# ohseokkwon/Foveated-Rendering-using-Ray-Tracing

Measured on AMD Instinct MI355X. Metric: Mrays/s + reconstructed fps @4K, 10% foveal density, 1/2/4/8 GPU, higher is better.
Workload: dtype f32

## Files before the change

### foveated-rendering-using-ray-tracing_amd/csrc/ctx_create.cpp

```cpp
#include <cmath>
#include <cstdlib>

#include "ctx_internal.h"

using namespace fr;
using fri::fail;

static thread_local std::string g_create_error;

int fri::fail(fr_ctx* c, int code, const std::string& msg) {
  if (c) c->err = msg; else g_create_error = msg;
  return code;
}

extern "C" {

const char* fr_version(void) { return "fovrt 0.2 (gfx950)"; }
int fr_abi_version(void) { return FOVRT_ABI_VERSION; }

int fr_config_default(fr_config* c) {
  if (!c) return FR_E_INVALID;
  memset(c, 0, sizeof(*c));
  c->abi_version = FOVRT_ABI_VERSION;
  c->width = 1024; c->height = 1024;
// ... 33 lines not shown
    const float M = std::max(v[0], std::max(v[1], v[2]));
    uint32_t word = 0;
    if (M > 0.0f) {
      int ex = 0;
      std::frexp(M, &ex);
      const int k = ex - 8, e = k + 136;
      if (e < 1 || e > 255) return FR_TEX_F32;
      const float f = std::ldexp(1.0f, e - 136);
      for (int c = 0; c < 3; c++) {
        const float m = std::ldexp(v[c], -k);
        if (!(m >= 0.0f && m <= 255.0f) || m != std::floor(m) || !same((float)(int)m * f, v[c])) return FR_TEX_F32;
        word |= (uint32_t)m << (8 * c);
      }
      word |= (uint32_t)e << 24;
    } else if (!(same(v[0], 0.0f) && same(v[1], 0.0f) && same(v[2], 0.0f))) {
      return FR_TEX_F32;
    }
    out[i] = word;
  }
  return FR_TEX_RGBE;
}

static void read_env_knobs(fr_ctx* c) {
  if (const char* v = getenv("FOVRT_SHADE_CHUNK_REFR")) c->chunk_refr = (uint32_t)std::max(0, atoi(v));
  if (const char* v = getenv("FOVRT_SHADE_XCD_BANDS")) c->xcd_bands = atoi(v) != 0;
  if (const char* v = getenv("FOVRT_SHADE_HANDOFF")) c->handoff = (uint32_t)std::min(std::max(atoi(v), 0), 2);
  if (const char* v = getenv("FOVRT_TEX_PACKING")) c->tex_packing = atoi(v) != 0;
  if (const char* v = getenv("FOVRT_JFA_LAZY_OUTPUTS")) c->lazy_jfa_outputs = atoi(v) != 0;
  if (const char* v = getenv("FOVRT_EARLY_SETUP")) c->early_setup = atoi(v) != 0;
  if (const char* v = getenv("FOVRT_EXTRA_LAZY")) c->extra_lazy = atoi(v) != 0;
  if (const char* v = getenv("FOVRT_SIB_STRIP")) c->sib_strip = atoi(v) != 0;
  if (const char* v = getenv("FOVRT_SLOTS")) c->nslots = std::max(2, std::min(fr_ctx::MAX_SLOTS, atoi(v)));
  {
    const char* v = getenv("FOVRT_SHADE_BLOCKS_PER_CU");
    const int full = fr::shade_max_blocks_per_cu();
    c->shade_blocks_per_cu = v ? std::max(1, std::min(full, atoi(v))) : full;
  }
  if (const char* v = getenv("FOVRT_JFA_XCD")) c->jfa_xcd = atoi(v);
  if (const char* v = getenv("FOVRT_JFA_REUSE")) c->jfa_reuse = atoi(v) != 0;
  if (const char* v = getenv("FOVRT_SIB_STRIP_MID")) c->sib_strip_mid = atoi(v);
  if (const char* v = getenv("FOVRT_ATROUS_ROWS2")) c->atrous_rows2 = atoi(v) != 0;
  if (const char* v = getenv("FOVRT_ATROUS_XCD")) c->atrous_xcd = atoi(v) != 0;
  if (const char* v = getenv("FOVRT_RAYQ_BLOCKS")) c->rayq_blocks = (uint32_t)std::max(0, atoi(v));
}

static std::vector<hipEvent_t*> timed_events(fr_ctx* c) {
  fr_ctx::StageEvents& t = c->tev;
  std::vector<hipEvent_t*> v = {&t.begin, &t.geometry, &t.sampling, &t.optimize, &t.shading, &t.end, &t.paths_begin,
                                &t.paths_end, &t.chain2_begin, &t.pullpush, &t.atrous, &t.chain1_begin, &t.jfa,
                                &t.sibson, &t.stage_begin, &t.stage_end, &c->ev_carry_fork, &c->ev_carry_done,
                                &c->ev_recon_fork, &c->ev_chain2_done, &c->ev_stream_join};
  for (auto& s : c->lat.ev)
    for (hipEvent_t* e : {&s.front_begin, &s.front_end, &s.jfa_end, &s.recon_end}) v.push_back(e);
  return v;
}

int fr_create(const fr_config* cfg_in, fr_ctx** out) {
  if (!out) return fail(nullptr, FR_E_INVALID, "out is NULL");
  *out = nullptr;
  fr_config cfg;
  if (cfg_in) cfg = *cfg_in; else fr_config_default(&cfg);
  if (cfg.abi_version != FOVRT_ABI_VERSION)
    return fail(nullptr, FR_E_INVALID, "fr_config.abi_version != FOVRT_ABI_VERSION (initialise it with fr_config_default)");
  if (cfg.width <= 0 || cfg.height <= 0 || cfg.width > 32767 || cfg.height > 32767)
    return fail(nullptr, FR_E_INVALID, "width/height out of range (1..32767)");
  if (!(cfg.spp == 1 || cfg.spp == 2 || cfg.spp == 4 || cfg.spp == 8))
    return fail(nullptr, FR_E_UNSUPPORTED, "spp must be 1, 2, 4 or 8");
  if (cfg.mask_mode < 0 || cfg.mask_mode > 4) return fail(nullptr, FR_E_INVALID, "bad mask_mode");
// ... 348 lines not shown
```

### foveated-rendering-using-ray-tracing_amd/csrc/ctx_frame.cpp

```cpp
#include <immintrin.h>
#include <sched.h>

#include <chrono>
#include <cmath>
#include <functional>

#include "ctx_internal.h"

using namespace fr;
using namespace fri;

namespace {
constexpr float kPollDeadlineMs = 10000.0f;
inline void cpu_relax() { _mm_pause(); }
hipError_t poll_event(hipEvent_t ev, float deadline_ms) {
  const auto t0 = std::chrono::steady_clock::now();
  for (uint32_t n = 1;; n++) {
    const hipError_t e = hipEventQuery(ev);
    if (e != hipErrorNotReady) return e;
    if ((n & 63u) == 0) {
      if (std::chrono::duration<float, std::milli>(std::chrono::steady_clock::now() - t0).count() > deadline_ms)
        return hipErrorNotReady;
      sched_yield();
    } else {
// ... 161 lines not shown
    if (int rc = enqueue_optimize(c, c->stream)) return rc;
  }
  c->front_done.consume(c->stream);
  hipEvent_t* kt = nullptr;
  if (c->kt_on) {
    const int i = c->kt_next;
    if (c->kt_pending == fr_ctx::KT_RING) { kt_harvest(c, i); c->kt_pending--; }
    kt = c->kt_ev[i];
    c->kt_next = (i + 1) % fr_ctx::KT_RING;
    c->kt_pending++;
    hipEventRecord(kt[0], c->stream);
  }
  if (c->setup_early) {
    c->aux_i ^= 1;
    c->aux = c->aux_p[c->aux_i];
    c->aux_seed = c->aux_seed_p[c->aux_i];
  }
  const bool early = c->setup_early;
  c->setup_early = false;
  const bool hv = c->pipeline_mode == FR_PIPELINE_LATENCY && c->early_setup && c->U.shard_count <= 1 && !c->U.front_need;
  hipEventRecord(c->ev_carry_fork, c->stream);
  hipStreamWaitEvent(c->carry_stream, c->ev_carry_fork, 0);
  launch_carry_history(c->U, c->mask, c->img[P_wgt(c)], c->img[c->hist_cache], c->img[c->hist_cur],
                       c->img[P_shd(c)], hv ? c->hvalid : nullptr, c->carry_stream);
  hipEventRecord(c->ev_carry_done, c->carry_stream);
  const uint32_t N = (uint32_t)((size_t)c->W * c->H);
  if (!early)
    launch_sample_setup(c->U, c->active, c->ray_count, N, c->img[P_wgt(c)], c->img[c->hist_cache], nullptr, c->aux,
                        c->aux_seed, c->stream);
  if (c->time_kernels) hipEventRecord(c->tev.paths_begin, c->stream);
  if (kt) hipEventRecord(kt[1], c->stream);
  launch_shade_paths(c->dsc, c->U, c->active, c->ray_count, N, c->img[P_wgt(c)], c->img[c->hist_cache],
                     c->shade_ctr, c->samples, c->sample_help, c->stats, c->aux, c->aux_seed, c->chunk_refr,
                     c->xcd_bands, c->handoff, c->shade_blocks_per_cu, c->item_store, c->stream);
  if (c->time_kernels) hipEventRecord(c->tev.paths_end, c->stream);
  if (kt) hipEventRecord(kt[2], c->stream);
  hipStreamWaitEvent(c->stream, c->ev_carry_done, 0);
  launch_shade_resolve(c->U, c->active, c->ray_count, N, c->img[P_wgt(c)], c->img[c->hist_cache], c->samples,
                       c->sample_help, c->img[c->hist_cur], c->img[P_shd(c)], c->shade_ctr, c->handoff,
                       c->shade_blocks_per_cu, c->U.shard_count > 1 ? c->shade_radiance : nullptr, c->stream);
  if (kt) hipEventRecord(kt[3], c->stream);
  c->trace_done[c->slot].record(c->stream);
  mark_set_read(c);
  int rc = check_launch(c);
  std::swap(c->hist_cur, c->hist_cache);
  c->hvalid_fresh = hv;
  std::swap(c->depth_cur, c->depth_cache);
  return rc;
}

static void materialize_jfa(fr_ctx* c, hipStream_t s) {
  if (!c->jfa_coord_owed) return;
  launch_jfa_coord(c->jfa_final, c->img[P_JFA_COLOR], c->img[P_JFA_COORD], c->W, c->H, s);
  c->jfa_coord_owed = false;
}

void fr_ctx::ExtraDebt::record(const fr_ctx* c) {
  U = c->U;
  sc = c->dsc;
  box = c->dev_box;
  depth = c->depth_cur;
  nrm = P_nrm(c);
  wgt = P_wgt(c);
}
void fr_ctx::ExtraDebt::settle(fr_ctx* c) {
  if (!owed) return;
  join_recon(c);
// ... 356 lines not shown
```

### foveated-rendering-using-ray-tracing_amd/csrc/ctx_internal.h

```cpp
#pragma once
#include <hip/hip_runtime.h>

#include <cstring>
#include <string>
#include <vector>

#include "../../include/fovrt.h"
#include "fr_device.h"
#include "k_launch.h"
#include "scene.h"

#define FR_MAX_SHARD_RANKS 64

using fr::f2;
using fr::f3;
using fr::u2;
using fr::f4;
using fr::BvhNode;
using fr::TriGeo;
using fr::TriShade;
using fr::DevMaterial;
using fr::DevTexture;
using fr::DevScene;
using fr::DevStats;
// ... 146 lines not shown
  bool fov_dirty = true, fov_reset = true, fov_on_device = false;
  fr::FovState* fov_st = nullptr;
  fr::FovState* h_fov = nullptr;
  const uint32_t* fov_count = nullptr;
  uint8_t* cmask = nullptr;
  bool cmask_on = false, cmask_set = false;
  Fence mask_taken, mask_read;
  unsigned long long* words = nullptr;
  uint32_t* counts = nullptr;
  uint32_t* offsets = nullptr;
  uint32_t* tiles = nullptr;
  uint32_t* ray_count = nullptr;
  uint32_t* active = nullptr;
  uint32_t* shade_ctr = nullptr;
  f4* samples = nullptr;
  unsigned long long* sample_help = nullptr;
  f4* item_store = nullptr;
  f4* aux = nullptr;
  uint32_t* aux_seed = nullptr;
  f4* aux_p[2] = {};
  uint32_t* aux_seed_p[2] = {};
  int aux_i = 0;
  unsigned long long* hvalid = nullptr;
  bool hvalid_fresh = false;
  bool setup_early = false;
  bool early_setup = true;
  fr::JfaState jfa = {};
  uint32_t jfa_gen = 0;
  bool jfa_force = true;
  bool jfa_reuse = true;
  uint32_t chunk_refr = 0;
  uint32_t xcd_bands = 1;
  uint32_t handoff = 1;
  int shade_blocks_per_cu = 0;
  int jfa_xcd = 1;
  int sib_strip_mid = 0;
  bool atrous_rows2 = true;
  int atrous_xcd = 1;
  float* ftab = nullptr;
  f4 *pull = nullptr, *push = nullptr, *snap = nullptr;
  f4 *sib_prefix = nullptr, *sib_blocks = nullptr;
  uint32_t* sib_wide = nullptr;
  uint32_t* sib_strips = nullptr;
  f4* sib_rowp = nullptr;
  bool sib_prefix_fresh = false;
  const u2* jfa_final = nullptr;
  bool jfa_coord_owed = false;
  bool lazy_jfa_outputs = true;
  struct ExtraDebt {
    bool owed = false;
    FrameUniforms U;
    DevScene sc;
    const float* box = nullptr;
    int depth = P_DEPTH_A, nrm = P_NORMAL, wgt = P_WEIGHT;
    void record(const fr_ctx* c);
    bool reads(int phys) const;
    void settle(fr_ctx* c);
  } extra;
  bool extra_lazy = true;
  int pp_S = 0;
  DevStats* stats = nullptr;
  FrameUniforms U;
  uint32_t accum = 0;
  bool light_pending = false;
  bool compacted = false;
  bool mask_dirty = false;
// ... 66 lines not shown
```

### foveated-rendering-using-ray-tracing_amd/csrc/k_launch.h

```cpp
#pragma once
#include <hip/hip_runtime.h>

#include <cstddef>
#include <cstdint>
#include <string>

#include "fr_device.h"

namespace fr {
void launch_gbuffer(const DevScene& sc, const FrameUniforms& U, f4* position, f4* normal, f4* depth, f4* diffuse,
                    f4* weight, uint8_t* gclass, DevStats* stats, const f3* cur_pos, const f3* prev_pos,
                    hipStream_t stream);
void launch_shade_paths(const DevScene& sc, const FrameUniforms& U, const uint32_t* active, const uint32_t* ray_count,
                        uint32_t max_active, const f4* weight, const f4* history_cache, uint32_t* chunk_ctr,
                        f4* samples, unsigned long long* help, DevStats* stats, f4* aux, uint32_t* aux_seed,
                        uint32_t chunk_refr, uint32_t xcd_bands, uint32_t handoff, int per_cu, f4* item_store,
                        hipStream_t stream);
int shade_max_blocks_per_cu();
size_t shade_item_store_f4(int per_cu);
void launch_sample_setup(const FrameUniforms& U, const uint32_t* active, const uint32_t* ray_count, uint32_t max_active,
                         const f4* weight, const f4* history_cache, const unsigned long long* hvalid, f4* aux,
                         uint32_t* aux_seed, hipStream_t stream);
void launch_shade_resolve(const FrameUniforms& U, const uint32_t* active, const uint32_t* ray_count,
                          uint32_t max_active, const f4* weight, const f4* history_cache, const f4* samples,
                          unsigned long long* help, f4* history_buffer, f4* shading, uint32_t* chunk_ctr,
                          uint32_t handoff, int per_cu, f4* radiance, hipStream_t stream);
size_t shade_counter_words();
size_t shade_fx_slots(uint32_t max_active, int spp, uint32_t handoff, int per_cu);
void launch_carry_history(const FrameUniforms& U, const uint8_t* mask, const f4* weight, const f4* history_cache,
                          f4* history_buffer, f4* shading, unsigned long long* hvalid, hipStream_t stream);
void launch_shard_pack_active(const uint32_t* active, const uint32_t* ray_count, uint32_t capacity, const f4* radiance,
                              f4* vals, uint32_t* idx, hipStream_t stream);
void launch_shard_unpack_active(const FrameUniforms& U, const f4* vals, const uint32_t* idx, uint32_t n, uint32_t npix,
                                const f4* weight, const f4* history_cache, f4* history_buffer, f4* shading,
                                hipStream_t stream);
void launch_vring_pack(const f4* hist, int W, int H, int T, const int32_t* tiles, int ntiles, uint32_t* out,
                       hipStream_t stream);
void launch_vring_unpack(const uint32_t* in, int W, int H, int T, const int32_t* tiles, int ntiles, f4* hist,
                         hipStream_t stream);
void launch_ray_queries(const DevScene& sc, const void* rays, const uint32_t* masks, uint32_t n, int kind, void* out,
                        RayQueryState* rq, const RayModels& rm, uint32_t max_blocks, hipStream_t stream);
#ifdef FR_STAMPS
void launch_trace_queries(const DevScene& sc, const f4* queries, uint32_t n, f4* hits, uint32_t* ctr,
                          hipStream_t stream, int kind);
void diag_record_queries(f4* buf, uint32_t cap, hipStream_t stream);
uint32_t diag_recorded_queries(hipStream_t stream);
void diag_sample_trace(uint32_t* srec, uint32_t scap, uint32_t* wrec, uint32_t wcap, hipStream_t stream);
#endif

void launch_sampling(const FrameUniforms& U, const DevScene& sc, const f4* position, const f4* depth,
                     const f4* depth_cache, f4* weight, const f4* normal, const f4* diffuse, f4* extra, uint8_t* mask,
// ... 139 lines not shown
```

### foveated-rendering-using-ray-tracing_amd/csrc/k_trace.hip

```cpp
#include <hip/hip_runtime.h>
#include <cstdlib>
#include "fr_device.h"
#include "k_launch.h"

namespace fr {

#ifndef TRACE_BLOCK
#define TRACE_BLOCK 128
#endif
#define BVH_STACK FR_BVH_STACK
#define ITEM_STACK 24

#ifdef FR_STAMPS
FR_DEV uint64_t stamp() {
  uint64_t t;
  __builtin_amdgcn_sched_barrier(0);
  asm volatile("s_memtime %0\n\ts_waitcnt lgkmcnt(0)" : "=s"(t)::"memory");
  __builtin_amdgcn_sched_barrier(0);
  return t;
}
#define STAMP(v) const uint64_t v = stamp()
#define STAMP_ADD(acc, v) acc += stamp() - v
#else
#define STAMP(v)
// ... 424 lines not shown
        long long sum;
        if (__builtin_add_overflow(old, v[k], &sum)) ovf |= v[k] > 0 ? 16u << k : 256u << k;
      }
    if ((flags & FX_NONFINITE) | ovf) atomicOr(rec + 3, (unsigned long long)((flags & FX_NONFINITE) | ovf));
  }
};
FR_DEV float fx_comp(long long v, unsigned long long fl, int k) {
  const bool nan = (fl >> k) & 1, pinf = (fl >> (4 + k)) & 1, ninf = (fl >> (8 + k)) & 1;
  if (nan || (pinf && ninf)) return __builtin_nanf("");
  if (pinf) return INFINITY;
  if (ninf) return -INFINITY;
  return (float)((double)v * (1.0 / FX_ONE));
}
FR_DEV f3 sample_value(const f4* samples, unsigned long long* help, uint32_t slot, bool fx) {
  if (!fx) return xyz(samples[slot]);
  const ulonglong2* r = reinterpret_cast<const ulonglong2*>(samples) + (size_t)slot * 2;
  const ulonglong2 r0 = r[0], r1 = r[1];
  long long v0 = (long long)r0.x, v1 = (long long)r0.y, v2 = (long long)r1.x;
  unsigned long long fl = r1.y;
  if (fl & FX_HELPED) {
    ulonglong2* h = reinterpret_cast<ulonglong2*>(help + (size_t)slot * 4);
    const ulonglong2 h0 = h[0], h1 = h[1];
    const long long hv[3] = {(long long)h0.x, (long long)h0.y, (long long)h1.x};
    if (__builtin_add_overflow(v0, hv[0], &v0)) fl |= hv[0] > 0 ? 16u : 256u;
    if (__builtin_add_overflow(v1, hv[1], &v1)) fl |= hv[1] > 0 ? 32u : 512u;
    if (__builtin_add_overflow(v2, hv[2], &v2)) fl |= hv[2] > 0 ? 64u : 1024u;
    fl |= h1.y;
    h[0] = make_ulonglong2(0ull, 0ull);
    h[1] = make_ulonglong2(0ull, 0ull);
  }
  return mk3(fx_comp(v0, fl, 0), fx_comp(v1, fl, 1), fx_comp(v2, fl, 2));
}

struct PathState {
  int n;
  ItemState it;
  SampleSum total;
  f3 qo, qd;
  float qtmax;
  bool qany;
  int phase;
  bool diffuse_kind, want_child;
  f3 Kd, pres, cdir, front;
  float pm, nDl, LnDl, Ldist, phong;
  uint32_t cseed, seed;
};

FR_DEV void path_begin(PathState& ps, f3 o, f3 d, uint32_t seed, Counters cnt) {
  ps.n = 0;
  ps.it = ItemState{mk3(1.0f), 0, 1.0f};
  ps.total.clear();
  ps.qo = o; ps.qd = d; ps.qtmax = INFINITY; ps.qany = false;
  ps.phase = PH_ITEM;
  ps.diffuse_kind = true; ps.want_child = false;
  ps.Kd = ps.pres = ps.cdir = ps.front = mk3(0.0f);
  ps.pm = 1.0f; ps.nDl = ps.LnDl = ps.Ldist = 0.0f; ps.phong = -1.0f;
  ps.cseed = 0; ps.seed = seed;
  cnt.inc(C_PRIMARY);
}

FR_DEV bool path_shade_step(const DevScene& sc, const FrameUniforms& U, PathState& ps, const ItemStack& items, Counters cnt,
                            const Hit& h, float atten, f3& total) {
  int& n = ps.n;
  ItemState& it = ps.it;
  f3& qo = ps.qo;
  f3& qd = ps.qd;
  float& qtmax = ps.qtmax;
  bool& qany = ps.qany;
  int& phase = ps.phase;
  bool& diffuse_kind = ps.diffuse_kind;
  bool& want_child = ps.want_child;
  f3& Kd = ps.Kd;
  f3& pres = ps.pres;
  f3& cdir = ps.cdir;
  f3& front = ps.front;
  float& pm = ps.pm;
  float& nDl = ps.nDl;
  float& LnDl = ps.LnDl;
  float& Ldist = ps.Ldist;
  float& phong = ps.phong;
  uint32_t& cseed = ps.cseed;
  const uint32_t seed = ps.seed;
  const f3 cutoff = mk3(0.34f, 0.55f, 0.85f);
  {
    bool pop = false;
    if (phase == PH_ITEM) {
      if (h.leaf < 0) {
        total += it.w * envmap_miss(sc, qd);
        pop = true;
      } else {
        SurfaceHit s = surface(sc, h, qo, qd);
        const int type = sc.mats[s.mat].type;
        Kd = kd_of(sc, s.mat, s.uv);
        if (type == MATL_REFRACTION) {
          const f3 hp = fma3(h.t, qd, qo);
          const f3 nrm = s.ns;
          const f3 i = qd;
          const f3 wk = it.w * Kd;
          float reflection = 1.0f;
          if (it.depth < U.refraction_max_depth) {
            int pushed = 0;
            Item child;
            f3 tdir;
            if (refract(tdir, i, nrm, 1.4f)) {
              float cos_theta = dotc(i, nrm);
              if (cos_theta < 0.0f) cos_theta = -cos_theta;
              else cos_theta = dotc(tdir, nrm);
              reflection = fresnel_schlick(cos_theta, 3.0f, 0.1f, 1.0f);
              float importance = it.importance * (1.0f - reflection) * luminance(mk3(1.0f));
              if (importance > 0.01f) {
                if (n < ITEM_STACK) { child = Item{hp, tdir, wk * ((1.0f - reflection) * mk3(1.0f)), it.depth + 1, importance}; pushed = 1; cnt.inc(C_REFR); }
                else cnt.inc(C_OVERFLOW);
              } else {
                total += wk * ((1.0f - reflection) * mk3(1.0f) * cutoff);
              }
            }
            f3 r = reflect(i, nrm);
            float importance = it.importance * reflection * luminance(mk3(1.0f));
            if (importance > 0.01f) {
              if (n + pushed < ITEM_STACK) {
                if (pushed) items.put(n++, child);
                child = Item{hp, r, wk * (reflection * mk3(1.0f)), it.depth + 1, importance};
                pushed = 1;
                cnt.inc(C_REFL);
              } else {
                cnt.inc(C_OVERFLOW);
              }
            } else {
              total += wk * (reflection * mk3(1.0f) * cutoff);
            }
            if (pushed) {
              it = ItemState{child.w, child.depth, child.importance};
              qo = child.o; qd = child.d; qtmax = INFINITY; qany = false;
              phase = PH_ITEM;
              return false;
            }
          } else {
            cnt.inc(C_TRUNC);
          }
          pop = true;
        } else {
          const f3 ff = faceforward_neg(s.ns, qd, s.ng);
          uint32_t sd = seed;
          const float z1 = rnd(sd);
          const float z2 = rnd(sd);
          front = s.front;
          LightSample ls = light_sample(sc, ff, front, z1, z2);
          nDl = ls.nDl; LnDl = ls.LnDl; Ldist = ls.Ldist;
          cseed = sd;
          diffuse_kind = type == MATL_DIFFUSE;
          if (diffuse_kind) {
            pm = 1.0f;
            want_child = it.depth < U.diffuse_max_depth - 1;
            if (want_child) cdir = onb_inverse_transform(ff, cosine_sample_hemisphere(z1, z2));
          } else {
            f3 H = normalizec(ls.L - qd);
            float nDh = dotc(ff, H);
            phong = nDh > 0.0f ? fx_pow(nDh, 88.0f) : -1.0f;
            const float rn = 0.05f;
            pm = fresnel_schlick(-dotc(ff, qd), 5.0f, rn, 1.0f);
            float importance = it.importance * luminance(mk3(pm));
            want_child = importance > 0.01f && it.depth < U.reflection_max_depth;
            if (want_child) cdir = reflect(qd, ff);
          }
          phase = PH_PARENT_SHADOW;
          if (nDl > 0.0f && LnDl > 0.0f) {
            cnt.inc(C_SHADOW);
            qo = front; qd = ls.L; qtmax = Ldist; qany = true;
            return false;
          }
          atten = 0.0f;
        }
      }
    }
    if (!pop && phase == PH_PARENT_SHADOW) {
      f3 S = mk3(0.0f);
      if (nDl > 0.0f && LnDl > 0.0f && atten > 0.0f) {
        const float weight = light_weight(sc, nDl, LnDl, Ldist);
        if (diffuse_kind) {
          S += sc.light_emission * weight * mk3(atten);
        } else {
          f3 Lc = sc.light_emission * weight * mk3(atten);
          S += Kd * nDl * Lc;
          if (phong >= 0.0f) S = fma3(Lc * mk3(1.0f), mk3(phong), S);
        }
      }
      pres = Kd * S;
      if (want_child) {
        cnt.inc(diffuse_kind ? C_BOUNCE : C_MIRROR);
        qo = front; qd = cdir; qtmax = INFINITY; qany = false;
        phase = PH_CHILD;
        return false;
      }
      total += it.w * pres;
      pop = true;
    } else if (!pop && phase == PH_CHILD) {
      bool lit = false;
      if (h.leaf >= 0) {
        SurfaceHit s = surface(sc, h, qo, qd);
        if (sc.mats[s.mat].type == MATL_DIFFUSE) {
          const f3 ff = faceforward_neg(s.ns, qd, s.ng);
          uint32_t sd = cseed;
          const float z1 = rnd(sd);
          const float z2 = rnd(sd);
          Kd = kd_of(sc, s.mat, s.uv);
          LightSample ls = light_sample(sc, ff, s.front, z1, z2);
          nDl = ls.nDl; LnDl = ls.LnDl; Ldist = ls.Ldist;
          if (nDl > 0.0f && LnDl > 0.0f) {
            cnt.inc(C_SHADOW);
            qo = s.front; qd = ls.L; qtmax = Ldist; qany = true;
            phase = PH_CHILD_SHADOW;
            lit = true;
          }
        }
      }
      if (lit) return false;
      total += it.w * (pres + mk3(pm) * mk3(0.0f));
      pop = true;
    } else if (!pop && phase == PH_CHILD_SHADOW) {
      f3 S = mk3(0.0f);
      if (atten > 0.0f) S += sc.light_emission * light_weight(sc, nDl, LnDl, Ldist) * mk3(atten);
      total += it.w * fma3(mk3(pm), Kd * S, pres);
      pop = true;
    }
    if (n == 0) return true;
    const Item nx = items.get(--n);
    it = ItemState{nx.w, nx.depth, nx.importance};
    qo = nx.o; qd = nx.d; qtmax = INFINITY; qany = false;
    phase = PH_ITEM;
    return false;
  }
}

FR_DEV bool path_shade(const DevScene& sc, const FrameUniforms& U, PathState& ps, const ItemStack& items, Counters cnt,
                       const Hit& h, float atten, bool fx) {
  f3 c = fx ? mk3(0.0f) : ps.total.as_float();
  const bool done = path_shade_step(sc, U, ps, items, cnt, h, atten, c);
  if (fx) ps.total.add(c);
  else ps.total.set_float(c);
  return done;
}

FR_DEV Hit trace_closest(const DevScene& sc, Stack st, f3 o, f3 d, float tmin, float tmax) {
  Hit h;
  float a;
  traverse(sc, st, o, d, tmin, tmax, false, h, a);
  return h;
}

FR_DEV void counters_begin(uint32_t* lds) {
  if (threadIdx.x < C_COUNT) lds[threadIdx.x] = 0;
  __syncthreads();
}
FR_DEV void counters_end(DevStats* stats, uint32_t* lds, bool gbuf) {
  __syncthreads();
  if (threadIdx.x < C_COUNT) {
    unsigned long long v = lds[threadIdx.x];
    if (v) {
      unsigned long long* dst;
      switch (threadIdx.x) {
        case C_PRIMARY: dst = gbuf ? &stats->gbuffer_primary : &stats->primary; break;
        case C_SHADOW: dst = &stats->shadow; break;
        case C_BOUNCE: dst = &stats->diffuse_bounce; break;
        case C_MIRROR: dst = &stats->mirror; break;
        case C_REFR: dst = &stats->refraction; break;
        case C_REFL: dst = &stats->reflection; break;
        case C_TRUNC: dst = &stats->truncated; break;
        default: dst = &stats->bvh_overflow; break;
      }
      atomicAdd(dst, v);
// ... 185 lines not shown
__device__ f4* g_rec = nullptr;
__device__ uint32_t g_rec_n = 0;
__device__ uint32_t g_rec_cap = 0;
FR_DEV void record_query(f3 o, f3 d, float tmax, bool any) {
  if (!g_rec) return;
  const uint32_t i = atomicAdd(&g_rec_n, 1u);
  if (i < g_rec_cap) {
    g_rec[2 * (size_t)i] = mk4(o, tmax);
    g_rec[2 * (size_t)i + 1] = mk4(d, any ? 1.0f : 0.0f);
  }
}
#define RECORD_QUERY(ps) record_query(ps.qo, ps.qd, ps.qtmax, ps.qany)
#else
#define RECORD_QUERY(ps)
#endif

#ifdef FR_STAMPS
__device__ uint32_t* g_srec = nullptr;
__device__ uint32_t g_srec_cap = 0;
__device__ uint32_t* g_wrec = nullptr;
__device__ uint32_t g_wrec_cap = 0;
FR_DEV uint32_t rtime() { return (uint32_t)__builtin_amdgcn_s_memrealtime(); }
#define DIAG(x) x
#else
#define DIAG(x)
#endif

#ifndef TRAV_UNROLL
#define TRAV_UNROLL 2
#endif
#ifndef SHADE_FIRST_STEP
#define SHADE_FIRST_STEP 1
#endif
#ifndef SHADE_WAVES
#define SHADE_WAVES 3
#endif
#ifndef SHADE_EXIT_T
#define SHADE_EXIT_T 8
#endif
#ifndef SHADE_EXIT_S
#define SHADE_EXIT_S 0
#endif
#ifndef SHADE_EXIT_REFR
#define SHADE_EXIT_REFR 20
#endif
__global__ __launch_bounds__(TRACE_BLOCK) __attribute__((amdgpu_waves_per_eu(SHADE_WAVES, SHADE_WAVES))) void k_shade_paths(DevScene sc, FrameUniforms U,
                                                             const uint32_t* __restrict__ active,
                                                             const uint32_t* __restrict__ ray_count,
                                                             const f4* __restrict__ weight,
                                                             const f4* __restrict__ history_cache,
                                                             uint32_t* __restrict__ chunk_ctr,
                                                             f4* __restrict__ samples, DevStats* stats,
                                                             const f4* __restrict__ aux,
                                                             const uint32_t* __restrict__ aux_seed,
                                                             uint32_t chunk_refr_fixed, uint32_t xcd_bands,
                                                             unsigned long long* __restrict__ help, uint32_t fx_below,
                                                             f4* __restrict__ item_store) {
  __shared__ int32_t lds_stack[BVH_STACK * TRACE_BLOCK];
  __shared__ uint32_t lds_cnt[C_COUNT];
  __shared__ BvhNode lds_root;
  Stack st{&lds_stack[threadIdx.x]};
  if (threadIdx.x < 32) reinterpret_cast<float*>(&lds_root)[threadIdx.x] = reinterpret_cast<const float*>(sc.nodes)[threadIdx.x];
  counters_begin(lds_cnt);
  Counters cnt{lds_cnt};
  const ItemStack items{item_store + (size_t)(blockIdx.x * TRACE_BLOCK + threadIdx.x) * 4, gridDim.x * TRACE_BLOCK * 4u};
  const uint32_t spp_shift = __builtin_ctz((uint32_t)U.spp);
  const uint32_t total = ray_count[0] * (uint32_t)U.spp;
  const uint32_t nrefr = min(ray_count[1] * (uint32_t)U.spp, total);
  const bool fx = total < fx_below;
  const uint32_t lanes = gridDim.x * TRACE_BLOCK;
  const uint32_t chunk_refr = chunk_refr_fixed ? chunk_refr_fixed
                              : total < 8 * lanes
                                  ? min(max(nrefr / (lanes / 64), 8u), (uint32_t)SHADE_CHUNK) & ~((uint32_t)U.spp - 1u)
                                  : SHADE_CHUNK;
  const uint32_t nsmall = (nrefr + chunk_refr - 1) / chunk_refr;
  const uint32_t nchunks = nsmall + (total - nrefr + SHADE_CHUNK - 1) / SHADE_CHUNK;
  uint32_t cb[5];
  cb[0] = 0; cb[4] = total;
#pragma unroll
  for (int c = 1; c < 4; c++) cb[c] = min(ray_count[c] * (uint32_t)U.spp, total);
  cb[1] = nrefr;
  auto part = [&](int c, uint32_t s) {
    const uint32_t len = (cb[c + 1] - cb[c]) >> spp_shift;
    return cb[c] + (uint32_t)(((uint64_t)len * s / SHADE_SHARDS) << spp_shift);
  };
  const uint32_t lane = threadIdx.x & 63;
  const float tmin = sc.scene_epsilon;
  const bool exit_early = SHADE_EXIT_T > 0 && (SHADE_EXIT_REFR == 0 || (!fx && (uint64_t)nrefr * SHADE_EXIT_REFR >= total));
  uint32_t shard = blockIdx.x & (SHADE_SHARDS - 1);
  uint32_t shards_left = SHADE_SHARDS;
  uint32_t q_next = 0, q_end = 0;
  int ls = L_IDLE;
  uint32_t slot = 0;
  PathState ps;
  TravState ts;
  uint64_t trav_cycles = 0, step_cycles = 0, refill_cycles = 0, total_cycles = 0;
#ifdef FR_STAMPS
  uint32_t n_visits = 0, n_wave_steps = 0;
  uint32_t d_q = 0, d_steps = 0, d_t0 = 0, w_done = 0;
  const uint32_t w_begin = rtime();
  uint32_t w_dry = 0;
#endif
  STAMP(t_begin);
  while (true) {
    STAMP(t_refill);
    unsigned long long idle = __ballot(ls == L_IDLE);
    while (idle && (q_next < q_end || shards_left)) {
      if (q_next >= q_end) {
        if (xcd_bands) {
        bool found = false;
        uint32_t j = 0;
        if (lane == 0) j = atomicAdd(&chunk_ctr[shard * SHADE_SHARD_STRIDE], 1u);
        j = __builtin_amdgcn_readfirstlane(j);
#pragma unroll
        for (int c = 0; c < 4; c++) {
          const uint32_t b = part(c, shard), e = part(c, shard + 1);
          const uint32_t ch = c == 0 ? chunk_refr : SHADE_CHUNK;
          const uint32_t n = (e - b + ch - 1) / ch;
          if (!found && j < n) {
            q_next = b + j * ch;
// ... 71 lines not shown
          ps.seed = xseed;
          trav_begin(ts, ps.qd, ps.qtmax);
          RECORD_QUERY(ps);
          DIAG(d_q = 1; d_steps = 0; d_t0 = rtime());
          ls = L_TRAV;
        }
      }
    }
    STAMP_ADD(refill_cycles, t_refill);
    if (!__ballot(ls != L_IDLE)) {
      if (!more) break;
      continue;
    }
    STAMP(t_tr);
    const bool traverse = !SHADE_FIRST_STEP || !__ballot(ls == L_READY);
    for (uint32_t pass = 0; traverse && __ballot(ls == L_TRAV) &&
                            (!exit_early || pass < SHADE_EXIT_S || __popcll(__ballot(ls == L_TRAV)) > SHADE_EXIT_T ||
                             !__ballot(ls == L_READY));
         pass++) {
#ifdef FR_STAMPS
      n_wave_steps++;
      if (ls == L_TRAV) n_visits++;
#endif
#pragma unroll
      for (int u = 0; u < TRAV_UNROLL; u++)
        if (ls == L_TRAV) {
          DIAG(d_steps++);
          if (trav_step(sc, st, ts, ps.qo, ps.qd, tmin, ps.qtmax, ps.qany)) ls = L_READY;
        }
    }
    STAMP_ADD(trav_cycles, t_tr);
    STAMP(t_step);
    if (ls == L_READY) {
      const bool fin = path_shade(sc, U, ps, items, cnt, ts.best, (float)ts.atten, fx);
      if (fin) {
        ps.total.flush(samples, help, slot, fx);
        ls = L_IDLE;
#ifdef FR_STAMPS
        if (g_srec && slot < g_srec_cap) {
          g_srec[4 * (size_t)slot] = d_q; g_srec[4 * (size_t)slot + 1] = d_steps;
          g_srec[4 * (size_t)slot + 2] = d_t0; g_srec[4 * (size_t)slot + 3] = rtime();
        }
        w_done++;
#endif
      } else {
        trav_begin(ts, ps.qd, ps.qtmax);
        RECORD_QUERY(ps);
        DIAG(d_q++);
        ls = L_TRAV;
        if (SHADE_FIRST_STEP && !root_hit(lds_root, ps.qo, ts.inv, tmin, ps.qtmax)) ls = L_READY;
      }
    }
    STAMP_ADD(step_cycles, t_step);
  }
  STAMP_ADD(total_cycles, t_begin);
#ifdef FR_STAMPS
  if (lane == 0) {
    atomicAdd(&stats->pad[0], (unsigned long long)total_cycles);
    atomicAdd(&stats->pad[1], (unsigned long long)refill_cycles);
    atomicAdd(&stats->pad[2], (unsigned long long)step_cycles);
    atomicAdd(&stats->pad[3], (unsigned long long)trav_cycles);
    atomicAdd(&stats->pad[5], (unsigned long long)n_wave_steps);
  }
  atomicAdd(&stats->pad[4], (unsigned long long)n_visits);
  {
    const uint32_t wid = (blockIdx.x * TRACE_BLOCK + threadIdx.x) >> 6;
    const uint32_t w_end = rtime();
// ... 346 lines not shown
  rec[4] = mk4(kd.x, kd.y, kd.z, __int_as_float(word));
}

static uint32_t ray_query_resident_blocks() { return 256u * 4u * RQ_WAVES / (TRACE_BLOCK / 64); }

void launch_ray_queries(const DevScene& sc, const void* rays, const uint32_t* masks, uint32_t n, int kind, void* out,
                        RayQueryState* rq, const RayModels& rm, uint32_t max_blocks, hipStream_t stream) {
  if (n == 0) return;
  uint32_t blocks = std::min((n + TRACE_BLOCK - 1) / TRACE_BLOCK, ray_query_resident_blocks());
  if (max_blocks) blocks = std::min(blocks, max_blocks);
  (void)hipMemsetAsync(rq, 0, sizeof(RayQueryState), stream);
  auto k = masks ? (kind == 1 ? k_ray_queries<1, true> : kind == 2 ? k_ray_queries<2, true> : k_ray_queries<0, true>)
                 : (kind == 1 ? k_ray_queries<1, false> : kind == 2 ? k_ray_queries<2, false> : k_ray_queries<0, false>);
  hipLaunchKernelGGL(k, dim3(blocks), dim3(TRACE_BLOCK), 0, stream, sc, static_cast<const f4*>(rays), n, out, rq, masks,
                     rm);
  if (kind == 2)
    hipLaunchKernelGGL(k_ray_surface, dim3((n + RS_BLOCK - 1) / RS_BLOCK), dim3(RS_BLOCK), 0, stream, sc,
                       static_cast<const f4*>(rays), n, static_cast<f4*>(out), rm);
}

void launch_gbuffer(const DevScene& sc, const FrameUniforms& U, f4* position, f4* normal, f4* depth, f4* diffuse,
                    f4* weight, uint8_t* gclass, DevStats* stats, const f3* cur_pos, const f3* prev_pos,
                    hipStream_t stream) {
  int tiles = ((U.width + 7) / 8) * ((U.height + 7) / 8);
  int threads = tiles * 64;
  int blocks = (threads + TRACE_BLOCK - 1) / TRACE_BLOCK;
  const bool motion = cur_pos && prev_pos;
  auto k = U.front_need ? (motion ? k_gbuffer<true, true> : k_gbuffer<true, false>)
                        : (motion ? k_gbuffer<false, true> : k_gbuffer<false, false>);
  hipLaunchKernelGGL(k, dim3(blocks), dim3(TRACE_BLOCK), 0, stream, sc, U, position, normal, depth, diffuse, weight,
                     gclass, stats, cur_pos, prev_pos);
}

int shade_max_blocks_per_cu() { return 4 * SHADE_WAVES / (TRACE_BLOCK / 64); }
static int shade_blocks(const FrameUniforms& U, uint32_t max_active, int per_cu) {
  size_t slots = (size_t)max_active * U.spp;
  return (int)std::min<size_t>((slots + TRACE_BLOCK - 1) / TRACE_BLOCK, (size_t)256 * per_cu);
}

static bool shade_fx_frame(int spp, uint32_t max_active, uint32_t handoff, int per_cu) {
  if (handoff == 0) return false;
  if (handoff >= 2) return true;
  FrameUniforms U{};
  U.spp = spp;
  const uint64_t lanes = (uint64_t)shade_blocks(U, max_active, per_cu) * TRACE_BLOCK;
  return (uint64_t)max_active * (uint64_t)spp < (uint64_t)SHADE_FX_FRAME * lanes;
}

size_t shade_fx_slots(uint32_t max_active, int spp, uint32_t handoff, int per_cu) {
  return shade_fx_frame(spp, max_active, handoff, per_cu) ? (size_t)max_active * spp : 0;
}

static uint32_t shade_fx_below(const FrameUniforms& U, uint32_t max_active, uint32_t handoff, int per_cu) {
  return shade_fx_frame(U.spp, max_active, handoff, per_cu) ? 0xFFFFFFFFu : 0u;
}

void launch_shade_paths(const DevScene& sc, const FrameUniforms& U, const uint32_t* active, const uint32_t* ray_count,
                        uint32_t max_active, const f4* weight, const f4* history_cache, uint32_t* chunk_ctr,
                        f4* samples, unsigned long long* help, DevStats* stats, f4* aux, uint32_t* aux_seed,
                        uint32_t chunk_refr, uint32_t xcd_bands, uint32_t handoff, int per_cu, f4* item_store,
                        hipStream_t stream) {
  if (max_active == 0) return;
  const int blocks = shade_blocks(U, max_active, per_cu);
  const uint32_t cr = chunk_refr ? std::min(std::max(chunk_refr & ~((uint32_t)U.spp - 1u), (uint32_t)U.spp), (uint32_t)SHADE_CHUNK) : 0u;
  const uint32_t fxb = shade_fx_below(U, max_active, handoff, per_cu);
  hipLaunchKernelGGL(k_shade_paths, dim3(blocks), dim3(TRACE_BLOCK), 0, stream, sc,
                     U, active, ray_count, weight, history_cache, chunk_ctr, samples, stats, aux, aux_seed, cr,
                     xcd_bands, help, fxb, item_store);
}

size_t shade_item_store_f4(int per_cu) {
  FrameUniforms U{};
  U.spp = 1;
  return (size_t)shade_blocks(U, 0xFFFFFFFFu, per_cu) * TRACE_BLOCK * ITEM_STACK * 4;
}

void launch_sample_setup(const FrameUniforms& U, const uint32_t* active, const uint32_t* ray_count, uint32_t max_active,
                         const f4* weight, const f4* history_cache, const unsigned long long* hvalid, f4* aux,
                         uint32_t* aux_seed, hipStream_t stream) {
  if (max_active == 0) return;
  hipLaunchKernelGGL(k_sample_setup, dim3((unsigned)std::min<size_t>((max_active + 255) / 256, 4096)), dim3(256), 0,
                     stream, U, active, ray_count, weight, history_cache, hvalid, aux, aux_seed);
}

void launch_shade_resolve(const FrameUniforms& U, const uint32_t* active, const uint32_t* ray_count,
                          uint32_t max_active, const f4* weight, const f4* history_cache, const f4* samples,
                          unsigned long long* help, f4* history_buffer, f4* shading, uint32_t* chunk_ctr,
                          uint32_t handoff, int per_cu, f4* radiance, hipStream_t stream) {
  if (max_active == 0) return;
  int rblocks = (int)std::min<size_t>((max_active + 255) / 256, 4096);
  hipLaunchKernelGGL(k_shade_resolve, dim3(rblocks), dim3(256), 0, stream, U, active, ray_count, weight,
                     history_cache, samples, history_buffer, shading, chunk_ctr, help,
                     shade_fx_below(U, max_active, handoff, per_cu), radiance);
}

size_t shade_counter_words() { return SHADE_SHARDS * SHADE_SHARD_STRIDE; }

void launch_carry_history(const FrameUniforms& U, const uint8_t* mask, const f4* weight, const f4* history_cache,
                          f4* history_buffer, f4* shading, unsigned long long* hvalid, hipStream_t stream) {
// ... 8 lines not shown
```

Before: 5340.

## Park path-shading state in LDS and add a 4-wave shade kernel variant

Moves per-path shading temporaries (Kd, pres, child direction, front, pm, nDl, LnDl) out of registers into a per-thread LDS park area, and templates the shade kernel on waves-per-EU. A host heuristic picks 4 waves when the slot count is large relative to the lane count, otherwise 3, and block counts per CU follow that choice. A scalar-register move for the epsilon is also forced. The aim is to lower VGPR pressure so more waves fit and latency is hidden better, at the cost of extra LDS traffic and more LDS per block, which may limit occupancy.

Result: slower. 5262 (-1.5%).

```diff
diff --git a/foveated-rendering-using-ray-tracing_amd/csrc/ctx_create.cpp b/foveated-rendering-using-ray-tracing_amd/csrc/ctx_create.cpp
--- a/foveated-rendering-using-ray-tracing_amd/csrc/ctx_create.cpp
+++ b/foveated-rendering-using-ray-tracing_amd/csrc/ctx_create.cpp
@@ -89,8 +89,10 @@
   if (const char* v = getenv("FOVRT_SIB_STRIP")) c->sib_strip = atoi(v) != 0;
   if (const char* v = getenv("FOVRT_SLOTS")) c->nslots = std::max(2, std::min(fr_ctx::MAX_SLOTS, atoi(v)));
   {
+    const char* w = getenv("FOVRT_SHADE_WAVES");
+    c->shade_waves = fr::shade_waves_for(w ? std::max(1, atoi(w)) : 0, (uint32_t)((size_t)c->W * c->H), c->cfg.spp);
     const char* v = getenv("FOVRT_SHADE_BLOCKS_PER_CU");
-    const int full = fr::shade_max_blocks_per_cu();
+    const int full = fr::shade_max_blocks_per_cu(c->shade_waves);
     c->shade_blocks_per_cu = v ? std::max(1, std::min(full, atoi(v))) : full;
   }
   if (const char* v = getenv("FOVRT_JFA_XCD")) c->jfa_xcd = atoi(v);
diff --git a/foveated-rendering-using-ray-tracing_amd/csrc/ctx_frame.cpp b/foveated-rendering-using-ray-tracing_amd/csrc/ctx_frame.cpp
--- a/foveated-rendering-using-ray-tracing_amd/csrc/ctx_frame.cpp
+++ b/foveated-rendering-using-ray-tracing_amd/csrc/ctx_frame.cpp
@@ -217,7 +217,7 @@
   if (kt) hipEventRecord(kt[1], c->stream);
   launch_shade_paths(c->dsc, c->U, c->active, c->ray_count, N, c->img[P_wgt(c)], c->img[c->hist_cache],
                      c->shade_ctr, c->samples, c->sample_help, c->stats, c->aux, c->aux_seed, c->chunk_refr,
-                     c->xcd_bands, c->handoff, c->shade_blocks_per_cu, c->item_store, c->stream);
+                     c->xcd_bands, c->handoff, c->shade_blocks_per_cu, c->shade_waves, c->item_store, c->stream);
   if (c->time_kernels) hipEventRecord(c->tev.paths_end, c->stream);
   if (kt) hipEventRecord(kt[2], c->stream);
   hipStreamWaitEvent(c->stream, c->ev_carry_done, 0);
diff --git a/foveated-rendering-using-ray-tracing_amd/csrc/ctx_internal.h b/foveated-rendering-using-ray-tracing_amd/csrc/ctx_internal.h
--- a/foveated-rendering-using-ray-tracing_amd/csrc/ctx_internal.h
+++ b/foveated-rendering-using-ray-tracing_amd/csrc/ctx_internal.h
@@ -202,6 +202,7 @@
   uint32_t chunk_refr = 0;
   uint32_t xcd_bands = 1;
   uint32_t handoff = 1;
+  int shade_waves = 0;
   int shade_blocks_per_cu = 0;
   int jfa_xcd = 1;
   int sib_strip_mid = 0;
diff --git a/foveated-rendering-using-ray-tracing_amd/csrc/k_launch.h b/foveated-rendering-using-ray-tracing_amd/csrc/k_launch.h
--- a/foveated-rendering-using-ray-tracing_amd/csrc/k_launch.h
+++ b/foveated-rendering-using-ray-tracing_amd/csrc/k_launch.h
@@ -14,9 +14,10 @@
 void launch_shade_paths(const DevScene& sc, const FrameUniforms& U, const uint32_t* active, const uint32_t* ray_count,
                         uint32_t max_active, const f4* weight, const f4* history_cache, uint32_t* chunk_ctr,
                         f4* samples, unsigned long long* help, DevStats* stats, f4* aux, uint32_t* aux_seed,
-                        uint32_t chunk_refr, uint32_t xcd_bands, uint32_t handoff, int per_cu, f4* item_store,
+                        uint32_t chunk_refr, uint32_t xcd_bands, uint32_t handoff, int per_cu, int waves, f4* item_store,
                         hipStream_t stream);
-int shade_max_blocks_per_cu();
+int shade_waves_for(int requested, uint32_t max_active, int spp);
+int shade_max_blocks_per_cu(int waves);
 size_t shade_item_store_f4(int per_cu);
 void launch_sample_setup(const FrameUniforms& U, const uint32_t* active, const uint32_t* ray_count, uint32_t max_active,
                          const f4* weight, const f4* history_cache, const unsigned long long* hvalid, f4* aux,
diff --git a/foveated-rendering-using-ray-tracing_amd/csrc/k_trace.hip b/foveated-rendering-using-ray-tracing_amd/csrc/k_trace.hip
--- a/foveated-rendering-using-ray-tracing_amd/csrc/k_trace.hip
+++ b/foveated-rendering-using-ray-tracing_amd/csrc/k_trace.hip
@@ -480,6 +480,15 @@
   return mk3(fx_comp(v0, fl, 0), fx_comp(v1, fl, 1), fx_comp(v2, fl, 2));
 }
 
+enum ParkId : int { P_KD = 0, P_PRES = 3, P_CDIR = 6, P_FRONT = 9, P_PM = 12, P_NDL = 13, P_LNDL = 14, PARK = 15 };
+struct Park {
+  float* base;
+  FR_DEV float get(int k) const { return base[k * TRACE_BLOCK]; }
+  FR_DEV void set(int k, float v) const { base[k * TRACE_BLOCK] = v; }
+  FR_DEV f3 get3(int k) const { return mk3(get(k), get(k + 1), get(k + 2)); }
+  FR_DEV void set3(int k, f3 v) const { set(k, v.x); set(k + 1, v.y); set(k + 2, v.z); }
+};
+
 struct PathState {
   int n;
   ItemState it;
@@ -489,8 +498,7 @@
   bool qany;
   int phase;
   bool diffuse_kind, want_child;
-  f3 Kd, pres, cdir, front;
-  float pm, nDl, LnDl, Ldist, phong;
+  float Ldist, phong;
   uint32_t cseed, seed;
 };
 
@@ -501,14 +509,13 @@
   ps.qo = o; ps.qd = d; ps.qtmax = INFINITY; ps.qany = false;
   ps.phase = PH_ITEM;
   ps.diffuse_kind = true; ps.want_child = false;
-  ps.Kd = ps.pres = ps.cdir = ps.front = mk3(0.0f);
-  ps.pm = 1.0f; ps.nDl = ps.LnDl = ps.Ldist = 0.0f; ps.phong = -1.0f;
+  ps.Ldist = 0.0f; ps.phong = -1.0f;
   ps.cseed = 0; ps.seed = seed;
   cnt.inc(C_PRIMARY);
 }
 
-FR_DEV bool path_shade_step(const DevScene& sc, const FrameUniforms& U, PathState& ps, const ItemStack& items, Counters cnt,
-                            const Hit& h, float atten, f3& total) {
+FR_DEV bool path_shade_step(const DevScene& sc, const FrameUniforms& U, PathState& ps, const Park park, const ItemStack& items,
+                            Counters cnt, const Hit& h, float atten, f3& total) {
   int& n = ps.n;
   ItemState& it = ps.it;
   f3& qo = ps.qo;
@@ -518,13 +525,6 @@
   int& phase = ps.phase;
   bool& diffuse_kind = ps.diffuse_kind;
   bool& want_child = ps.want_child;
-  f3& Kd = ps.Kd;
-  f3& pres = ps.pres;
-  f3& cdir = ps.cdir;
-  f3& front = ps.front;
-  float& pm = ps.pm;
-  float& nDl = ps.nDl;
-  float& LnDl = ps.LnDl;
   float& Ldist = ps.Ldist;
   float& phong = ps.phong;
   uint32_t& cseed = ps.cseed;
@@ -539,7 +539,7 @@
       } else {
         SurfaceHit s = surface(sc, h, qo, qd);
         const int type = sc.mats[s.mat].type;
-        Kd = kd_of(sc, s.mat, s.uv);
+        const f3 Kd = kd_of(sc, s.mat, s.uv);
         if (type == MATL_REFRACTION) {
           const f3 hp = fma3(h.t, qd, qo);
           const f3 nrm = s.ns;
@@ -592,24 +592,28 @@
           uint32_t sd = seed;
           const float z1 = rnd(sd);
           const float z2 = rnd(sd);
-          front = s.front;
+          const f3 front = s.front;
           LightSample ls = light_sample(sc, ff, front, z1, z2);
-          nDl = ls.nDl; LnDl = ls.LnDl; Ldist = ls.Ldist;
+          const float nDl = ls.nDl, LnDl = ls.LnDl;
+          Ldist = ls.Ldist;
+          park.set3(P_KD, Kd); park.set3(P_FRONT, front);
+          park.set(P_NDL, nDl); park.set(P_LNDL, LnDl);
           cseed = sd;
           diffuse_kind = type == MATL_DIFFUSE;
           if (diffuse_kind) {
-            pm = 1.0f;
+            park.set(P_PM, 1.0f);
             want_child = it.depth < U.diffuse_max_depth - 1;
-            if (want_child) cdir = onb_inverse_transform(ff, cosine_sample_hemisphere(z1, z2));
+            if (want_child) park.set3(P_CDIR, onb_inverse_transform(ff, cosine_sample_hemisphere(z1, z2)));
           } else {
             f3 H = normalizec(ls.L - qd);
             float nDh = dotc(ff, H);
             phong = nDh > 0.0f ? fx_pow(nDh, 88.0f) : -1.0f;
             const float rn = 0.05f;
-            pm = fresnel_schlick(-dotc(ff, qd), 5.0f, rn, 1.0f);
+            const float pm = fresnel_schlick(-dotc(ff, qd), 5.0f, rn, 1.0f);
+            park.set(P_PM, pm);
             float importance = it.importance * luminance(mk3(pm));
             want_child = importance > 0.01f && it.depth < U.reflection_max_depth;
-            if (want_child) cdir = reflect(qd, ff);
+            if (want_child) park.set3(P_CDIR, reflect(qd, ff));
           }
           phase = PH_PARENT_SHADOW;
           if (nDl > 0.0f && LnDl > 0.0f) {
@@ -623,6 +627,8 @@
     }
     if (!pop && phase == PH_PARENT_SHADOW) {
       f3 S = mk3(0.0f);
+      const f3 Kd = park.get3(P_KD);
+      const float nDl = park.get(P_NDL), LnDl = park.get(P_LNDL);
       if (nDl > 0.0f && LnDl > 0.0f && atten > 0.0f) {
         const float weight = light_weight(sc, nDl, LnDl, Ldist);
         if (diffuse_kind) {
@@ -633,10 +639,11 @@
           if (phong >= 0.0f) S = fma3(Lc * mk3(1.0f), mk3(phong), S);
         }
       }
-      pres = Kd * S;
+      const f3 pres = Kd * S;
       if (want_child) {
+        park.set3(P_PRES, pres);
         cnt.inc(diffuse_kind ? C_BOUNCE : C_MIRROR);
-        qo = front; qd = cdir; qtmax = INFINITY; qany = false;
+        qo = park.get3(P_FRONT); qd = park.get3(P_CDIR); qtmax = INFINITY; qany = false;
         phase = PH_CHILD;
         return false;
       }
@@ -651,10 +658,13 @@
           uint32_t sd = cseed;
           const float z1 = rnd(sd);
           const float z2 = rnd(sd);
-          Kd = kd_of(sc, s.mat, s.uv);
+          const f3 Kd = kd_of(sc, s.mat, s.uv);
           LightSample ls = light_sample(sc, ff, s.front, z1, z2);
-          nDl = ls.nDl; LnDl = ls.LnDl; Ldist = ls.Ldist;
+          const float nDl = ls.nDl, LnDl = ls.LnDl;
+          Ldist = ls.Ldist;
           if (nDl > 0.0f && LnDl > 0.0f) {
+            park.set3(P_KD, Kd);
+            park.set(P_NDL, nDl); park.set(P_LNDL, LnDl);
             cnt.inc(C_SHADOW);
             qo = s.front; qd = ls.L; qtmax = Ldist; qany = true;
             phase = PH_CHILD_SHADOW;
@@ -663,12 +673,12 @@
         }
       }
       if (lit) return false;
-      total += it.w * (pres + mk3(pm) * mk3(0.0f));
+      total += it.w * (park.get3(P_PRES) + mk3(park.get(P_PM)) * mk3(0.0f));
       pop = true;
     } else if (!pop && phase == PH_CHILD_SHADOW) {
       f3 S = mk3(0.0f);
-      if (atten > 0.0f) S += sc.light_emission * light_weight(sc, nDl, LnDl, Ldist) * mk3(atten);
-      total += it.w * fma3(mk3(pm), Kd * S, pres);
+      if (atten > 0.0f) S += sc.light_emission * light_weight(sc, park.get(P_NDL), park.get(P_LNDL), Ldist) * mk3(atten);
+      total += it.w * fma3(mk3(park.get(P_PM)), park.get3(P_KD) * S, park.get3(P_PRES));
       pop = true;
     }
     if (n == 0) return true;
@@ -680,10 +690,10 @@
   }
 }
 
-FR_DEV bool path_shade(const DevScene& sc, const FrameUniforms& U, PathState& ps, const ItemStack& items, Counters cnt,
-                       const Hit& h, float atten, bool fx) {
+FR_DEV bool path_shade(const DevScene& sc, const FrameUniforms& U, PathState& ps, const Park park, const ItemStack& items,
+                       Counters cnt, const Hit& h, float atten, bool fx) {
   f3 c = fx ? mk3(0.0f) : ps.total.as_float();
-  const bool done = path_shade_step(sc, U, ps, items, cnt, h, atten, c);
+  const bool done = path_shade_step(sc, U, ps, park, items, cnt, h, atten, c);
   if (fx) ps.total.add(c);
   else ps.total.set_float(c);
   return done;
@@ -935,9 +945,8 @@
 #ifndef SHADE_FIRST_STEP
 #define SHADE_FIRST_STEP 1
 #endif
-#ifndef SHADE_WAVES
-#define SHADE_WAVES 3
-#endif
+#define SHADE_WAVES_MIN 3
+#define SHADE_WAVES_MAX 4
 #ifndef SHADE_EXIT_T
 #define SHADE_EXIT_T 8
 #endif
@@ -947,7 +956,8 @@
 #ifndef SHADE_EXIT_REFR
 #define SHADE_EXIT_REFR 20
 #endif
-__global__ __launch_bounds__(TRACE_BLOCK) __attribute__((amdgpu_waves_per_eu(SHADE_WAVES, SHADE_WAVES))) void k_shade_paths(DevScene sc, FrameUniforms U,
+template <int WAVES>
+__global__ __launch_bounds__(TRACE_BLOCK) __attribute__((amdgpu_waves_per_eu(WAVES, WAVES))) void k_shade_paths(DevScene sc, FrameUniforms U,
                                                              const uint32_t* __restrict__ active,
                                                              const uint32_t* __restrict__ ray_count,
                                                              const f4* __restrict__ weight,
@@ -962,7 +972,12 @@
   __shared__ int32_t lds_stack[BVH_STACK * TRACE_BLOCK];
   __shared__ uint32_t lds_cnt[C_COUNT];
   __shared__ BvhNode lds_root;
+  __shared__ float lds_park[PARK * TRACE_BLOCK];
+  static_assert(sizeof(lds_stack) + sizeof(lds_cnt) + sizeof(lds_root) + sizeof(lds_park) <=
+                    160 * 1024 / (4 * SHADE_WAVES_MAX / (TRACE_BLOCK / 64)),
+                "k_shade_paths: the block's LDS does not fit SHADE_WAVES_MAX waves per SIMD");
   Stack st{&lds_stack[threadIdx.x]};
+  const Park park{&lds_park[threadIdx.x]};
   if (threadIdx.x < 32) reinterpret_cast<float*>(&lds_root)[threadIdx.x] = reinterpret_cast<const float*>(sc.nodes)[threadIdx.x];
   counters_begin(lds_cnt);
   Counters cnt{lds_cnt};
@@ -988,7 +1003,8 @@
     return cb[c] + (uint32_t)(((uint64_t)len * s / SHADE_SHARDS) << spp_shift);
   };
   const uint32_t lane = threadIdx.x & 63;
-  const float tmin = sc.scene_epsilon;
+  float tmin;
+  asm("s_mov_b32 %0, %1" : "=s"(tmin) : "s"(sc.scene_epsilon));
   const bool exit_early = SHADE_EXIT_T > 0 && (SHADE_EXIT_REFR == 0 || (!fx && (uint64_t)nrefr * SHADE_EXIT_REFR >= total));
   uint32_t shard = blockIdx.x & (SHADE_SHARDS - 1);
   uint32_t shards_left = SHADE_SHARDS;
@@ -1126,7 +1142,7 @@
     STAMP_ADD(trav_cycles, t_tr);
     STAMP(t_step);
     if (ls == L_READY) {
-      const bool fin = path_shade(sc, U, ps, items, cnt, ts.best, (float)ts.atten, fx);
+      const bool fin = path_shade(sc, U, ps, park, items, cnt, ts.best, (float)ts.atten, fx);
       if (fin) {
         ps.total.flush(samples, help, slot, fx);
         ls = L_IDLE;
@@ -1539,7 +1555,7 @@
                      gclass, stats, cur_pos, prev_pos);
 }
 
-int shade_max_blocks_per_cu() { return 4 * SHADE_WAVES / (TRACE_BLOCK / 64); }
+int shade_max_blocks_per_cu(int waves) { return 4 * waves / (TRACE_BLOCK / 64); }
 static int shade_blocks(const FrameUniforms& U, uint32_t max_active, int per_cu) {
   size_t slots = (size_t)max_active * U.spp;
   return (int)std::min<size_t>((slots + TRACE_BLOCK - 1) / TRACE_BLOCK, (size_t)256 * per_cu);
@@ -1554,6 +1570,18 @@
   return (uint64_t)max_active * (uint64_t)spp < (uint64_t)SHADE_FX_FRAME * lanes;
 }
 
+#define SHADE_W4_FX 8
+#define SHADE_W4_FP 192
+int shade_waves_for(int requested, uint32_t max_active, int spp) {
+  if (requested) return std::max(SHADE_WAVES_MIN, std::min(SHADE_WAVES_MAX, requested));
+  FrameUniforms U{};
+  U.spp = spp;
+  const uint64_t slots = (uint64_t)max_active * (uint64_t)spp;
+  const uint64_t lanes4 = (uint64_t)shade_blocks(U, max_active, shade_max_blocks_per_cu(SHADE_WAVES_MAX)) * TRACE_BLOCK;
+  const bool fx = shade_fx_frame(spp, max_active, 1u, shade_max_blocks_per_cu(SHADE_WAVES_MIN));
+  return slots >= (uint64_t)(fx ? SHADE_W4_FX : SHADE_W4_FP) * lanes4 ? SHADE_WAVES_MAX : SHADE_WAVES_MIN;
+}
+
 size_t shade_fx_slots(uint32_t max_active, int spp, uint32_t handoff, int per_cu) {
   return shade_fx_frame(spp, max_active, handoff, per_cu) ? (size_t)max_active * spp : 0;
 }
@@ -1565,13 +1593,13 @@
 void launch_shade_paths(const DevScene& sc, const FrameUniforms& U, const uint32_t* active, const uint32_t* ray_count,
                         uint32_t max_active, const f4* weight, const f4* history_cache, uint32_t* chunk_ctr,
                         f4* samples, unsigned long long* help, DevStats* stats, f4* aux, uint32_t* aux_seed,
-                        uint32_t chunk_refr, uint32_t xcd_bands, uint32_t handoff, int per_cu, f4* item_store,
+                        uint32_t chunk_refr, uint32_t xcd_bands, uint32_t handoff, int per_cu, int waves, f4* item_store,
                         hipStream_t stream) {
   if (max_active == 0) return;
   const int blocks = shade_blocks(U, max_active, per_cu);
   const uint32_t cr = chunk_refr ? std::min(std::max(chunk_refr & ~((uint32_t)U.spp - 1u), (uint32_t)U.spp), (uint32_t)SHADE_CHUNK) : 0u;
   const uint32_t fxb = shade_fx_below(U, max_active, handoff, per_cu);
-  hipLaunchKernelGGL(k_shade_paths, dim3(blocks), dim3(TRACE_BLOCK), 0, stream, sc,
+  hipLaunchKernelGGL(waves == SHADE_WAVES_MAX ? k_shade_paths<4> : k_shade_paths<3>, dim3(blocks), dim3(TRACE_BLOCK), 0, stream, sc,
                      U, active, ray_count, weight, history_cache, chunk_ctr, samples, stats, aux, aux_seed, cr,
                      xcd_bands, help, fxb, item_store);
 }
```
